# KaffinPX/neptune-core

Hardware: AMD Instinct MI355X
Metric: STARK proofs verified/sec (whole node) + Tip5 perms/sec vs VALU roofline (higher is better)
Workload: dtype u64 (Goldilocks mod p; XFE = cubic extension)

## Files before the change

neptune-core_amd/csrc/stark_kernels.hip:

```cpp
#include <hip/hip_ext.h>

#include <atomic>
#include <cstdlib>

#include "../../include/nhip_challenge_id.h"
#include "kernels.hpp"
#include "proof_codec.hpp"
#include "stark.hpp"
#include "stark_launch_plan.hpp"
#include "tip5_device.hpp"
#include "xfe.hpp"

namespace nhip {

#ifndef NHIP_LAT_PRIO
#define NHIP_LAT_PRIO 2
#endif
__device__ __forceinline__ void latency_priority() {
    if constexpr (NHIP_LAT_PRIO > 0) __builtin_amdgcn_s_setprio(NHIP_LAT_PRIO);
}
__device__ uint32_t g_batches_done;
struct AgePrio {
    uint32_t seq, k;
};
__device__ __forceinline__ void age_priority(AgePrio a, int base) {
    bool old = false;
    if (a.k) {
        const uint32_t done = __builtin_amdgcn_readfirstlane(
            __hip_atomic_load(&g_batches_done, __ATOMIC_RELAXED, __HIP_MEMORY_SCOPE_AGENT));
        old = (int32_t)(a.seq - done) < (int32_t)a.k;
    }
    switch (base + (old ? 1 : 0)) {
        case 0: break;
        case 1: __builtin_amdgcn_s_setprio(1); break;
        case 2: __builtin_amdgcn_s_setprio(2); break;
        default: __builtin_amdgcn_s_setprio(3); break;
// ... 213 lines not shown
                if (f + e < nwords) xs[xcur + f + e] = s[0];
                if (f + 4 + e < nwords) xs[xcur + f + 4 + e] = s[1];
                if (r2 && f + 8 + e < nwords) xs[xcur + f + 8 + e] = s[2];
                tip5_permute_quad(s, cq, rck, e, lds.lut);
            }
            xcur += nwords;
        } else {
            const uint64_t bound = op.arg;
            uint32_t got = 0;
            while (got < op.n) {
                const uint64_t v0 = from_mont(s[0]), v1 = from_mont(s[1]), v2 = from_mont(s[2]);
                tip5_permute_quad(s, cq, rck, e, lds.lut);
                const bool ok0 = v0 != GL_P - 1, ok1 = v1 != GL_P - 1, ok2 = r2 && v2 != GL_P - 1;
                const uint64_t b0 = __ballot(ok0), b1 = __ballot(ok1), b2 = __ballot(ok2);
                const uint32_t bits = ((uint32_t)(b0 >> qb) & 0xFu) | (((uint32_t)(b1 >> qb) & 0xFu) << 4) |
                                      (((uint32_t)(b2 >> qb) & 0x3u) << 8);
                auto put = [&](bool ok, uint32_t w, uint64_t v) {
                    const uint32_t rank = __popc(bits & ((1u << w) - 1u));
                    if (ok && got + rank < op.n) idx_out[icur + got + rank] = (uint32_t)((v & 0xFFFFFFFFull) % bound);
                };
                put(ok0, e, v0);
                put(ok1, 4 + e, v1);
                put(ok2, 8 + e, v2);
                got += __popc(bits);
            }
            icur += op.n;
        }
    }
}

#ifndef NHIP_ROWS_WAVES
#define NHIP_ROWS_WAVES 5
#endif
template <bool MW>
__global__ void __launch_bounds__(256, NHIP_ROWS_WAVES) k_hash_rows(const uint64_t* __restrict__ words, const ProofDesc* __restrict__ desc,
                                                   uint32_t n_proofs, uint32_t k, StarkDims dims,
                                                   uint64_t* __restrict__ dig, const uint32_t* __restrict__ fail,
                                                   AgePrio age) {
    age_priority(age, 0);
    __shared__ Tip5Lds lds;
    tip5_lds_init(lds);
    const uint32_t tree = blockIdx.y;
    const uint32_t width = tree == 0 ? dims.num_main : (tree == 1 ? 3 * dims.num_aux : 3 * dims.num_quot_seg);
    for (uint64_t t = blockIdx.x * (uint64_t)blockDim.x + threadIdx.x; t < (uint64_t)n_proofs * k;
         t += (uint64_t)gridDim.x * blockDim.x) {
        const uint32_t p = (uint32_t)(t / k), j = (uint32_t)(t % k);
        if (fail[p]) continue;
        const ProofDesc& d = desc[p];
        const uint64_t base = (tree == 0 ? d.main_rows_off : (tree == 1 ? d.aux_rows_off : d.quot_rows_off)) +
                              (uint64_t)j * width;
        const uint64_t* __restrict__ row = words + base;
        uint64_t s[16];
#pragma unroll
        for (int q = 0; q < 16; ++q) s[q] = 0;
        const uint32_t nchunks = width / TIP5_RATE + 1;
        for (uint32_t c = 0; c < nchunks; ++c) {
            const uint32_t pos = c * TIP5_RATE;
            const bool last = c + 1 == nchunks;
            if (!last) {
#pragma unroll
                for (int q = 0; q < TIP5_RATE; ++q) s[q] = word_mont<MW>(row[pos + q]);
            } else {
                const uint32_t rem = width - pos;
#pragma unroll
                for (int q = 0; q < TIP5_RATE; ++q) {
                    const uint32_t qq = (uint32_t)q;
                    s[q] = qq < rem ? word_mont<MW>(row[pos + qq]) : (qq == rem ? MONT_ONE : 0ull);
                }
            }
            tip5_rounds_0_3(s, lds.lut);
            tip5_last_sbox(s, lds.lut);
            if (!last) tip5_last_mds<10, 16>(s);
            else tip5_last_mds<0, 5>(s);
        }
        uint64_t* __restrict__ o = dig + (((uint64_t)p * 3 + tree) * k + j) * 5;
#pragma unroll
        for (int q = 0; q < 5; ++q) o[q] = s[q];
    }
}

template <bool MW>
__device__ __forceinline__ void hash_rows_wide_body(uint32_t bx, uint32_t tree, const Tip5Lds& t5,
                                                    const uint64_t* __restrict__ words,
                                                    const ProofDesc* __restrict__ desc, uint32_t n_proofs,
                                                    uint32_t k, StarkDims dims, uint64_t* __restrict__ dig,
                                                    const uint32_t* __restrict__ fail) {
    const uint32_t width = tree == 0 ? dims.num_main : (tree == 1 ? 3 * dims.num_aux : 3 * dims.num_quot_seg);
    const uint32_t e = threadIdx.x & 15u;
    const uint64_t t = ((uint64_t)bx * blockDim.x + threadIdx.x) >> 4;
    if (t >= (uint64_t)n_proofs * k) return;
    const uint32_t p = (uint32_t)(t / k), j = (uint32_t)(t % k);
    if (fail[p]) return;
    const ProofDesc& d = desc[p];
    const uint64_t* __restrict__ row =
        words + (tree == 0 ? d.main_rows_off : (tree == 1 ? d.aux_rows_off : d.quot_rows_off)) + (uint64_t)j * width;
    uint64_t rcs[TIP5_ROUNDS];
#pragma unroll
    for (int r = 0; r < TIP5_ROUNDS; ++r) rcs[r] = c_tip5_rc_raw[r * 16 + e];
    const uint32_t nchunks = width / TIP5_RATE + 1;
    auto chunk_word = [&](uint32_t c) -> uint64_t {
        const uint32_t pos = c * TIP5_RATE;
        if (c + 1 < nchunks) return e < TIP5_RATE ? word_mont<MW>(row[pos + e]) : 0ull;
        const uint32_t rem = width - pos;
// ... 299 lines not shown
                                               unsigned long long* __restrict__ perm_counter) {
    latency_priority();
    mp_plan_body<B>(blockIdx.x, blockIdx.y, words, desc, n_proofs, k, trees_per_proof, dig, idx_all, plan, fail,
                    perm_counter);
}

struct LcwTree {
    uint64_t* nodes;
    uint32_t max_len;
};

template <bool MW>
__device__ __forceinline__ void lcw_node(const uint64_t* __restrict__ words, const ProofDesc& d,
                                         const uint64_t* __restrict__ mine, uint32_t v, uint32_t L, uint64_t o[5]) {
    if (v >= L) {
        const uint64_t off = d.last_cw_off + 3ull * (v - L);
        o[0] = word_mont<MW>(words[off]);
        o[1] = word_mont<MW>(words[off + 1]);
        o[2] = word_mont<MW>(words[off + 2]);
        o[3] = 0;
        o[4] = 0;
    } else {
#pragma unroll
        for (int q = 0; q < 5; ++q) o[q] = mine[5ull * v + q];
    }
}

#ifndef NHIP_MP_WAVES
#define NHIP_MP_WAVES 6
#endif
#ifndef NHIP_MP_WAVES_SMALL
#define NHIP_MP_WAVES_SMALL 7
#endif
template <int WAVES, bool MW>
__global__ void __launch_bounds__(256, WAVES) k_mp_hash(const uint64_t* __restrict__ words, const uint64_t* __restrict__ dig,
                                                 MpPlan plan, uint32_t lvl, uint32_t mp_blocks,
                                                 const ProofDesc* __restrict__ desc, uint32_t n_proofs,
                                                 const uint32_t* __restrict__ fail, LcwTree lcw, AgePrio age) {
    __shared__ Tip5Lds t5;
    __shared__ uint64_t s_base[MP_SHARDS + 1];
    __shared__ uint32_t s_cnt[MP_SHARDS];
    age_priority(age, NHIP_MP_PRIO);
    const bool is_lcw = blockIdx.x >= mp_blocks;
    if (!is_lcw) {
        if (threadIdx.x < MP_SHARDS) {
            s_base[threadIdx.x] = plan.shard_base[lvl * MP_SHARDS + threadIdx.x];
            s_cnt[threadIdx.x] = plan.counter[lvl * MP_SHARDS + threadIdx.x];
        }
        if (threadIdx.x == 0)
            s_base[MP_SHARDS] = plan.shard_base[(lvl + 1) * MP_SHARDS - 1] + plan.shard_cap[(lvl + 1) * MP_SHARDS - 1];
    }
    tip5_lds_init(t5);
    uint64_t s[16];
    uint64_t* o = nullptr;
    bool work = false;
    if (is_lcw) {
        const uint32_t per = lcw.max_len >> (lvl + 1);
        const uint64_t q = (uint64_t)(blockIdx.x - mp_blocks) * blockDim.x + threadIdx.x;
        const uint32_t p = (uint32_t)(q / per), i = (uint32_t)(q % per);
        if (p < n_proofs && !(fail[p] & FAIL_DECODE)) {
            const ProofDesc& d = desc[p];
            const uint32_t L = d.last_cw_n;
            if (i < (L >> (lvl + 1))) {
                const uint32_t v = (L >> (lvl + 1)) + i;
                uint64_t* mine = lcw.nodes + (uint64_t)p * lcw.max_len * 5;
                lcw_node<MW>(words, d, mine, 2 * v, L, s);
                lcw_node<MW>(words, d, mine, 2 * v + 1, L, s + 5);
                o = mine + 5ull * v;
                work = true;
            }
        }
    } else {
        const uint64_t g = s_base[0] + (uint64_t)blockIdx.x * blockDim.x + threadIdx.x;
        if (g < s_base[MP_SHARDS]) {
            uint32_t sh = 0;
#pragma unroll
            for (uint32_t q = 1; q < MP_SHARDS; ++q) sh += g >= s_base[q] ? 1u : 0u;
            if (g - s_base[sh] < s_cnt[sh]) {
                const uint64_t lc = plan.ops[2 * g], rc = plan.ops[2 * g + 1];
                if (lc != MPS_NONE) {
                    mp_load<MW>(lc, words, dig, plan.arena, s);
                    mp_load<MW>(rc, words, dig, plan.arena, s + 5);
                    o = plan.arena + 5 * g;
                    work = true;
                }
            }
        }
    }
    if (!work) return;
    tip5_hash_pair_digest(s, t5.lut);
#pragma unroll
    for (int q = 0; q < 5; ++q) o[q] = s[q];
}

template <bool MW>
__device__ __forceinline__ uint64_t mp_load_word(uint64_t code, uint32_t e, const uint64_t* __restrict__ words,
                                                 const uint64_t* __restrict__ dig, const uint64_t* __restrict__ arena) {
    const uint64_t t = code >> 62, v = code & MPS_MASK;
    if (t == MPS_ARENA) return arena[5 * v + e];
    if (t == MPS_DIG) return dig[5 * v + e];
    if (t == MPS_AUTH) return word_mont<MW>(words[v + e]);
    return e < 3 ? word_mont<MW>(words[v + e]) : 0ull;
}

template <bool MW>
__device__ __forceinline__ uint64_t lcw_node_word(const uint64_t* __restrict__ words, const ProofDesc& d,
                                                  const uint64_t* __restrict__ mine, uint32_t v, uint32_t L, uint32_t e) {
    if (v >= L) return e < 3 ? word_mont<MW>(words[d.last_cw_off + 3ull * (v - L) + e]) : 0ull;
    return mine[5ull * v + e];
}

template <bool MW>
__global__ void __launch_bounds__(256) k_mp_hash_wide(const uint64_t* __restrict__ words,
                                                      const uint64_t* __restrict__ dig, MpPlan plan, uint32_t lvl,
                                                      uint64_t mp_rows, const ProofDesc* __restrict__ desc,
                                                      uint32_t n_proofs, const uint32_t* __restrict__ fail, LcwTree lcw) {
    latency_priority();
    __shared__ Tip5Lds t5;
    __shared__ uint64_t s_base[MP_SHARDS + 1];
    __shared__ uint32_t s_cnt[MP_SHARDS];
    if (threadIdx.x < MP_SHARDS) {
        s_base[threadIdx.x] = plan.shard_base[lvl * MP_SHARDS + threadIdx.x];
        s_cnt[threadIdx.x] = plan.counter[lvl * MP_SHARDS + threadIdx.x];
// ... 827 lines not shown
        hipLaunchKernelGGL(k_fs_rows_small<MW>, dim3(p.fs_grid), dim3(p.fs_block), 0, sa, b.words, b.desc, b.ops, n, b.xs,
                           b.idx, b.fail, age_sponge, p.fs_blocks, p.rows_gx, k, b.dims, b.dig);
    else if (p.fs_form == FS_PAIR)
        hipLaunchKernelGGL((k_fs_replay_wide<true, MW>), dim3(p.fs_grid), dim3(p.fs_block), 0, sa, b.words, b.desc, b.ops,
                           n, b.xs, b.idx, b.fail, age_sponge);
    else if (p.fs_form == FS_QUAD)
        hipLaunchKernelGGL(k_fs_replay_quad<MW>, dim3(p.fs_grid), dim3(p.fs_block), 0, sa, b.words, b.desc, b.ops, n,
                           b.xs, b.idx, b.fail, age_sponge);
    else
        hipLaunchKernelGGL((k_fs_replay_wide<false, MW>), dim3(p.fs_grid), dim3(p.fs_block), 0, sa, b.words, b.desc,
                           b.ops, n, b.xs, b.idx, b.fail, age_sponge);
    pad(sa);
    mark(EV_FS_DONE, sa);
    if (p.fused_plan_fri) {
        mark(EV_FRI_START, sa);
        hipLaunchKernelGGL(k_plan_fri_small<MW>, dim3(n * p.plan_groups + n), dim3(256), 0, sa, b.words, b.desc, n, k,
                           tpp, p.plan_groups, b.dig, b.idx, b.mp, b.fail, b.counters + CNT_MP_SKIPPED, b.dims, b.xs,
                           b.xdom);
    } else if (p.plan_block == 128) {
        hipLaunchKernelGGL(k_mp_plan<128>, dim3(n, p.plan_groups), dim3(128), 0, sa, b.words, b.desc, n, k, tpp, b.dig,
                           b.idx, b.mp, b.fail, b.counters + CNT_MP_SKIPPED);
    } else {
        hipLaunchKernelGGL(k_mp_plan<256>, dim3(n, p.plan_groups), dim3(256), 0, sa, b.words, b.desc, n, k, tpp, b.dig,
                           b.idx, b.mp, b.fail, b.counters + CNT_MP_SKIPPED);
    }
    pad(sa);
    mark(EV_PLAN_DONE, sa);
    if (!p.fused_fs_rows) {
        hipEvent_t r0 = p.rows_timed ? tm->rev[0] : nullptr, r1 = p.rows_timed ? tm->rev[1] : nullptr;
        if (p.rows_wide)
            launch_ev(k_hash_rows_wide<MW>, dim3(p.rows_grid, 3), dim3(256), 0, st, r0, r1, b.words, b.desc, n, k, b.dims,
                      b.dig, b.fail);
        else
            launch_ev(k_hash_rows<MW>, dim3(p.rows_grid, 3), dim3(256), 0, st, r0, r1, b.words, b.desc, n, k, b.dims,
                      b.dig, b.fail, age);
    }
    pad(st);
    mark(EV_ROWS_DONE, st);
    auto fri = [&](hipStream_t s) {
        hipLaunchKernelGGL(k_fri<MW>, dim3(n), dim3(256), 0, s, b.words, b.desc, n, b.dims, b.xs, b.idx, b.xdom, b.fail);
    };
    if (p.fri_on_main) {
        if (!p.fused_plan_fri) {
            wait(st, EV_FS_DONE);
            mark(EV_FRI_START, st);
            fri(st);
            pad(st);
        }
        mark(EV_FRI_DONE, st);
    }
    wait(st, EV_PLAN_DONE);
    auto aux_chain = [&]() {
        mark(EV_AUX_RELEASE, st);
        if (!p.fri_on_main) wait(sa, EV_AUX_RELEASE);
        mark(EV_AUX_START, sa);
        if (p.ood_block == 1024) {
            if (p.ood_global_slots) ood(k_ood_air<1024, MW, true>);
            else ood(k_ood_air<1024, MW, false>);
        } else {
            if (p.ood_global_slots) ood(k_ood_air<256, MW, true>);
            else ood(k_ood_air<256, MW, false>);
        }
        pad(sa);
        mark(EV_OOD_DONE, sa);
        if (p.fri_on_main) {
            wait(sa, EV_FRI_DONE);
        } else {
            fri(sa);
            mark(EV_FRI_DONE, sa);
        }
        hipLaunchKernelGGL(k_deep_rows8<MW>, dim3(n), dim3(256), deep_rows8_lds_bytes(b.dims), sa, b.words, b.desc, n,
                           b.dims, b.xs, b.xdom, b.ood, b.fail);
        pad(sa);
        mark(EV_DEEP_DONE, sa);
    };
    auto climb = [&](const HashStep& h) {
        launch_ev(k_mp_climb<MW>, dim3(h.grid, tpp + 1), dim3(MP_CLIMB_THREADS), 0, st, timed(h, 0), timed(h, 1), b.words,
                  b.dig, b.mp, tpp, b.desc, n, (const uint32_t*)b.fail, lcw, h.level);
    };
    for (uint32_t s = 0; s < p.n_steps; ++s) {
        if (s == p.aux_release_step) aux_chain();
        const HashStep& h = p.steps[s];
        switch (h.kind) {
            case HashKind::Climb: climb(h); break;
            case HashKind::Tail: {
                TailCaps caps{};
                for (uint32_t t = 0; t < MP_TAIL_LEVELS_MAX; ++t) caps.cap[t] = p.tail_caps[t];
                launch_ev(k_mp_hash_tail<MW>, dim3(h.grid), dim3(MP_TAIL_THREADS), 0, st, timed(h, 0), timed(h, 1), b.words,
                          b.dig, b.mp, h.level, p.hash_levels, caps, b.desc, n, (const uint32_t*)b.fail, lcw);
                break;
            }
            case HashKind::Wide:
                launch_ev(k_mp_hash_wide<MW>, dim3(h.grid), dim3(256), 0, st, timed(h, 0), timed(h, 1), b.words, b.dig,
                          b.mp, h.level, h.arg, b.desc, n, (const uint32_t*)b.fail, lcw);
                break;
            case HashKind::Level7:
                launch_ev((k_mp_hash<NHIP_MP_WAVES_SMALL, MW>), dim3(h.grid), dim3(256), 0, st, timed(h, 0), timed(h, 1),
                          b.words, b.dig, b.mp, h.level, (uint32_t)h.arg, b.desc, n, (const uint32_t*)b.fail, lcw, age);
                break;
            case HashKind::Level6:
                launch_ev((k_mp_hash<NHIP_MP_WAVES, MW>), dim3(h.grid), dim3(256), 0, st, timed(h, 0), timed(h, 1),
                          b.words, b.dig, b.mp, h.level, (uint32_t)h.arg, b.desc, n, (const uint32_t*)b.fail, lcw, age);
                break;
        }
    }
    if (p.one_climb) pad(st);
    if (p.aux_release_step == p.n_steps) aux_chain();
    mark(EV_HASH_DONE, st);
    if (p.roots_one_launch) {
        hipLaunchKernelGGL(k_roots_verdicts_small<MW>, dim3(p.roots_grid), dim3(ROOTS_ONE_WG), 0, st, b.words, b.desc,
                           b.dig, b.mp, p.n_records, tpp, k, b.fail, n, lcw, b.verdicts);
        mark(EV_ROOTS_DONE, st);
    } else {
        hipLaunchKernelGGL(k_mp_roots<MW>, dim3(p.roots_grid), dim3(256), 0, st, b.words, b.desc, b.dig, b.mp,
                           p.n_records, tpp, k, b.fail, n, lcw);
        pad(st);
        mark(EV_ROOTS_DONE, st);
        wait(st, EV_DEEP_DONE);
        hipLaunchKernelGGL(k_verdicts, dim3(p.verdicts_grid), dim3(256), 0, st, b.fail, n, b.verdicts);
    }
    mark(EV_VERDICTS, st);
    return hipGetLastError();
}

hipError_t launch_stark_phases(const StarkBatchDev& b, hipStream_t st, hipStream_t sa, StarkPhaseTimer* tm) {
    return b.D.mont_words ? launch_phases<true>(b, st, sa, tm) : launch_phases<false>(b, st, sa, tm);
}

template <bool MW>
static hipError_t set_attributes() {
    for (const void* f : {(const void*)k_ood_air<256, MW, false>, (const void*)k_ood_air<256, MW, true>,
                          (const void*)k_ood_air<1024, MW, false>, (const void*)k_ood_air<1024, MW, true>}) {
        const hipError_t e = hipFuncSetAttribute(f, hipFuncAttributeMaxDynamicSharedMemorySize, AIR_LDS_BUDGET);
        if (e != hipSuccess) return e;
// ... 12 lines not shown
```

neptune-core_amd/csrc/stark_launch_plan.hpp:

```cpp
#pragma once
#include <cstdint>
#include <cstdlib>

#include "ab_env.hpp"
#include "kernels.hpp"

namespace nhip {

static constexpr uint32_t MP_CLIMB_MAX_PROOFS = 32;
static constexpr uint32_t ROWS_WIDE_MAX_PROOFS = 32;
static constexpr uint32_t OOD_WIDE_MAX_PROOFS = 64;
static constexpr uint32_t FS_PAIR_MAX_PROOFS = 512;
static constexpr uint32_t FS_QUAD_MIN_PROOFS = 2048;
static constexpr uint32_t FS_QUAD_WG = 256;
static constexpr uint32_t MP_SMALL_MAX_PROOFS = 4096;
static constexpr uint64_t MP_WIDE_MAX_OPS = 48 * 1024;
#ifndef NHIP_MP_TAIL_MAX_OPS
#define NHIP_MP_TAIL_MAX_OPS 256
#endif
static constexpr uint64_t MP_TAIL_MAX_OPS = NHIP_MP_TAIL_MAX_OPS;
static constexpr uint32_t CLIMB_FROM_MIN_LEVELS = 24;
static constexpr uint64_t CLIMB_FROM_OPS_DEFAULT = 4096;
static constexpr uint32_t CLIMB_FROM_MIN_REST = 3;
static constexpr uint32_t AUX_AFTER_LEVEL_DEFAULT = 0;
static constexpr uint32_t AGE_PRIO_OLDEST = 2;
static constexpr uint32_t AGE_PRIO_MIN_PROOFS = 2048;

enum FsForm { FS_ROW = 0, FS_PAIR = 1, FS_QUAD = 2 };

struct LaunchKnobs {
    uint32_t ood_wide_max = OOD_WIDE_MAX_PROOFS;
    uint32_t rows_wide_max = ROWS_WIDE_MAX_PROOFS;
    uint32_t quad_wg = FS_QUAD_WG;
    uint32_t quad_min = FS_QUAD_MIN_PROOFS;
    int fs_form_init = -1;
    int64_t age_prio = -1;
    bool age_prio_fs = false;
    bool fuse_fs_rows = true;
    bool fuse_plan_fri = true;
    uint32_t mp_small_max = MP_SMALL_MAX_PROOFS;
    uint32_t climb_max = MP_CLIMB_MAX_PROOFS;
    uint32_t aux_after_level = AUX_AFTER_LEVEL_DEFAULT;
    int pad_packets = 0;
};

inline unsigned long ab_unsigned(const char* name, unsigned long dflt) {
    const char* e = ab_env(name);
    return e ? std::strtoul(e, nullptr, 10) : dflt;
}

inline LaunchKnobs launch_knobs_from_env() {
    LaunchKnobs kn;
    kn.ood_wide_max = (uint32_t)ab_unsigned("NHIP_OOD_WIDE_MAX", kn.ood_wide_max);
    kn.rows_wide_max = (uint32_t)ab_unsigned("NHIP_ROWS_WIDE_MAX", kn.rows_wide_max);
    const uint32_t w = (uint32_t)ab_unsigned("NHIP_QUAD_WG", FS_QUAD_WG);
    kn.quad_wg = (w >= 64 && w <= 1024 && w % 64 == 0) ? w : FS_QUAD_WG;
    kn.quad_min = (uint32_t)ab_unsigned("NHIP_FS_QUAD_MIN", kn.quad_min);
    if (const char* v = ab_env("NHIP_FS_FORM"))
        kn.fs_form_init = v[0] == 'q' ? (int)FS_QUAD : v[0] == 'p' ? (int)FS_PAIR : v[0] == 'r' ? (int)FS_ROW : -1;
    kn.age_prio = (int64_t)ab_unsigned("NHIP_AGE_PRIO", (unsigned long)-1);
    if (const char* e = ab_env("NHIP_AGE_PRIO_FS")) kn.age_prio_fs = e[0] == '1';
    if (const char* e = ab_env("NHIP_FUSE_SMALL")) kn.fuse_fs_rows = e[0] != '0';
    if (const char* e = ab_env("NHIP_FUSE_PLAN_FRI")) kn.fuse_plan_fri = e[0] != '0';
    kn.mp_small_max = (uint32_t)ab_unsigned("NHIP_MP_SMALL_MAX", kn.mp_small_max);
    kn.climb_max = (uint32_t)ab_unsigned("NHIP_CLIMB_MAX", kn.climb_max);
    kn.aux_after_level = (uint32_t)ab_unsigned("NHIP_AUX_AFTER_LEVEL", kn.aux_after_level);
    kn.pad_packets = (int)ab_unsigned("NHIP_PAD_PACKETS", 0);
    return kn;
}
inline const LaunchKnobs& launch_knobs() {
    static const LaunchKnobs kn = launch_knobs_from_env();
    return kn;
}

static constexpr uint32_t event_bit(StarkEvent e) { return 1u << (int)e; }
static constexpr uint32_t CROSS_STREAM_EVENTS = event_bit(EV_FORK) | event_bit(EV_DECODED) | event_bit(EV_FS_DONE) |
                                                event_bit(EV_PLAN_DONE) | event_bit(EV_FRI_DONE) |
                                                event_bit(EV_AUX_RELEASE) | event_bit(EV_DEEP_DONE);
static constexpr uint32_t ALL_EVENTS = (1u << STARK_EVENTS) - 1;

struct LaunchInput {
    uint32_t n, k, max_R;
    uint32_t mp_levels;
    const uint64_t* mp_cap_host;
    uint32_t max_lcw;
    bool global_slots;
    uint32_t air_block;
    bool two_streams;
    bool phase_marks;
    bool launch_events;
    bool hash_events;
    int fs_form_forced;
    int64_t climb_from_forced;
};

enum class HashKind : uint8_t {
    Level6,
    Level7,
    Wide,
    Tail,
// ... 155 lines not shown
```

neptune-core_amd/csrc/tip5_device.hpp:

```cpp
#pragma once
#include "goldilocks.hpp"
#include "tip5_constants.h"

namespace nhip {

static constexpr int TIP5_STATE = 16;
static constexpr int TIP5_RATE = 10;
static constexpr int TIP5_ROUNDS = 5;
static constexpr uint64_t MONT_ONE = 0x00000000FFFFFFFFull;

__constant__ static uint64_t c_tip5_rc_raw[80] = {
#define NHIP_RC(i) TIP5_RC_RAW[i]
    NHIP_RC(0), NHIP_RC(1), NHIP_RC(2), NHIP_RC(3), NHIP_RC(4), NHIP_RC(5), NHIP_RC(6), NHIP_RC(7),
    NHIP_RC(8), NHIP_RC(9), NHIP_RC(10), NHIP_RC(11), NHIP_RC(12), NHIP_RC(13), NHIP_RC(14), NHIP_RC(15),
    NHIP_RC(16), NHIP_RC(17), NHIP_RC(18), NHIP_RC(19), NHIP_RC(20), NHIP_RC(21), NHIP_RC(22), NHIP_RC(23),
    NHIP_RC(24), NHIP_RC(25), NHIP_RC(26), NHIP_RC(27), NHIP_RC(28), NHIP_RC(29), NHIP_RC(30), NHIP_RC(31),
    NHIP_RC(32), NHIP_RC(33), NHIP_RC(34), NHIP_RC(35), NHIP_RC(36), NHIP_RC(37), NHIP_RC(38), NHIP_RC(39),
    NHIP_RC(40), NHIP_RC(41), NHIP_RC(42), NHIP_RC(43), NHIP_RC(44), NHIP_RC(45), NHIP_RC(46), NHIP_RC(47),
    NHIP_RC(48), NHIP_RC(49), NHIP_RC(50), NHIP_RC(51), NHIP_RC(52), NHIP_RC(53), NHIP_RC(54), NHIP_RC(55),
    NHIP_RC(56), NHIP_RC(57), NHIP_RC(58), NHIP_RC(59), NHIP_RC(60), NHIP_RC(61), NHIP_RC(62), NHIP_RC(63),
    NHIP_RC(64), NHIP_RC(65), NHIP_RC(66), NHIP_RC(67), NHIP_RC(68), NHIP_RC(69), NHIP_RC(70), NHIP_RC(71),
    NHIP_RC(72), NHIP_RC(73), NHIP_RC(74), NHIP_RC(75), NHIP_RC(76), NHIP_RC(77), NHIP_RC(78), NHIP_RC(79),
#undef NHIP_RC
};

__constant__ static uint64_t c_tip5_rck_raw[80] = {
#define NHIP_RC(i) (TIP5_RC_RAW[i] + 0xFFFFFFFFull)
    NHIP_RC(0), NHIP_RC(1), NHIP_RC(2), NHIP_RC(3), NHIP_RC(4), NHIP_RC(5), NHIP_RC(6), NHIP_RC(7),
    NHIP_RC(8), NHIP_RC(9), NHIP_RC(10), NHIP_RC(11), NHIP_RC(12), NHIP_RC(13), NHIP_RC(14), NHIP_RC(15),
    NHIP_RC(16), NHIP_RC(17), NHIP_RC(18), NHIP_RC(19), NHIP_RC(20), NHIP_RC(21), NHIP_RC(22), NHIP_RC(23),
    NHIP_RC(24), NHIP_RC(25), NHIP_RC(26), NHIP_RC(27), NHIP_RC(28), NHIP_RC(29), NHIP_RC(30), NHIP_RC(31),
    NHIP_RC(32), NHIP_RC(33), NHIP_RC(34), NHIP_RC(35), NHIP_RC(36), NHIP_RC(37), NHIP_RC(38), NHIP_RC(39),
    NHIP_RC(40), NHIP_RC(41), NHIP_RC(42), NHIP_RC(43), NHIP_RC(44), NHIP_RC(45), NHIP_RC(46), NHIP_RC(47),
    NHIP_RC(48), NHIP_RC(49), NHIP_RC(50), NHIP_RC(51), NHIP_RC(52), NHIP_RC(53), NHIP_RC(54), NHIP_RC(55),
    NHIP_RC(56), NHIP_RC(57), NHIP_RC(58), NHIP_RC(59), NHIP_RC(60), NHIP_RC(61), NHIP_RC(62), NHIP_RC(63),
// ... 180 lines not shown
#endif
template <int NIN, int OBEG, int OEND, int G>
__device__ __forceinline__ void mds_fold_groups(const uint32_t* lo, const uint32_t* hi,
                                                const uint64_t* __restrict__ rck, uint64_t* out) {
    constexpr int N = (OEND - OBEG) < G ? (OEND - OBEG) : G;
    mds_fold_outputs<NIN, OBEG, N>(lo, hi, rck, out);
    if constexpr (OBEG + N < OEND) {
        __builtin_amdgcn_sched_barrier(0);
        mds_fold_groups<NIN, OBEG + N, OEND, G>(lo, hi, rck, out + N);
    }
}

template <int NIN, int OBEG = 0, int OEND = 16, int G = 16>
__device__ __forceinline__ void mds_ark_fold(uint64_t s[16], const uint64_t* __restrict__ rck) {
    uint32_t lo[NIN], hi[NIN];
#pragma unroll
    for (int j = 0; j < NIN; ++j) {
        lo[j] = (uint32_t)s[j];
        hi[j] = (uint32_t)(s[j] >> 32);
    }
    uint64_t out[OEND - OBEG];
    mds_fold_groups<NIN, OBEG, OEND, G>(lo, hi, rck, out);
#pragma unroll
    for (int o = 0; o < OEND - OBEG; ++o) s[OBEG + o] = out[o];
}

template <int G = NHIP_SPONGE_MDS_GROUP>
__device__ __forceinline__ void mds_ark(uint64_t s[16], const uint64_t* __restrict__ rc,
                                        const uint64_t* __restrict__ rck) {
    (void)rc;
    mds_ark_fold<16, 0, 16, G>(s, rck);
}

__device__ __forceinline__ void tip5_permute_raw(uint64_t s[16], const uint8_t* __restrict__ lut) {
#pragma unroll 1
    for (int r = 0; r < TIP5_ROUNDS; ++r) {
#pragma unroll
        for (int i = 0; i < 4; ++i) s[i] = split_and_lookup(lut, s[i]);
        pow7_12(s + 4);
        mds_ark(s, c_tip5_rc_raw + r * 16, c_tip5_rck_raw + r * 16);
    }
}


__host__ __device__ constexpr uint64_t tip5_rck0_fixed(int i) {
    uint64_t k = TIP5_RC_RAW[i] + 0xFFFFFFFFull;
    for (int j = 10; j < 16; ++j) k += (uint64_t)TIP5_MDS[(i - j) & 15] * 0xFFFFFFFFull;
    return k;
}
constexpr bool tip5_rck0_fixed_in_range() {
    for (int i = 0; i < 16; ++i)
        if (tip5_rck0_fixed(i) >= 0xFFF0000000000000ull || tip5_rck0_fixed(i) < TIP5_RC_RAW[i]) return false;
    return true;
}
static_assert(tip5_rck0_fixed_in_range(), "round-0 FixedLength accumulator start below 2^64 - 2^52");
__constant__ static uint64_t c_tip5_rck0_fixed[16] = {
    tip5_rck0_fixed(0),  tip5_rck0_fixed(1),  tip5_rck0_fixed(2),  tip5_rck0_fixed(3),
    tip5_rck0_fixed(4),  tip5_rck0_fixed(5),  tip5_rck0_fixed(6),  tip5_rck0_fixed(7),
    tip5_rck0_fixed(8),  tip5_rck0_fixed(9),  tip5_rck0_fixed(10), tip5_rck0_fixed(11),
    tip5_rck0_fixed(12), tip5_rck0_fixed(13), tip5_rck0_fixed(14), tip5_rck0_fixed(15),
};

__device__ __forceinline__ void tip5_hash_pair_digest(uint64_t s[16], const uint8_t* __restrict__ lut) {
#pragma unroll
    for (int i = 0; i < 4; ++i) s[i] = split_and_lookup(lut, s[i]);
#pragma unroll
    for (int g = 4; g < 10; g += 3) {
        uint64_t x2[3], x4[3], x3[3];
        pow7_mul<3>(s + g, s + g, x2);
        pow7_mul<3>(x2, x2, x4);
        pow7_mul<3>(s + g, x2, x3);
        pow7_mul<3>(x3, x4, s + g);
    }
    mds_ark_fold<10, 0, 16, NHIP_PAIR_MDS_GROUP>(s, c_tip5_rck0_fixed);
#pragma unroll 1
    for (int r = 1; r < TIP5_ROUNDS - 1; ++r) {
#pragma unroll
        for (int i = 0; i < 4; ++i) s[i] = split_and_lookup(lut, s[i]);
        pow7_12(s + 4);
        mds_ark<NHIP_PAIR_MDS_GROUP>(s, c_tip5_rc_raw + r * 16, c_tip5_rck_raw + r * 16);
    }
#pragma unroll
    for (int i = 0; i < 4; ++i) s[i] = split_and_lookup(lut, s[i]);
    pow7_12(s + 4);
    mds_ark_fold<16, 0, 5, NHIP_PAIR_MDS_GROUP>(s, c_tip5_rck_raw + (TIP5_ROUNDS - 1) * 16);
}

__device__ __forceinline__ void tip5_rounds_0_3(uint64_t s[16], const uint8_t* __restrict__ lut) {
#pragma unroll 1
    for (int r = 0; r < TIP5_ROUNDS - 1; ++r) {
#pragma unroll
        for (int i = 0; i < 4; ++i) s[i] = split_and_lookup(lut, s[i]);
        pow7_12(s + 4);
        mds_ark(s, c_tip5_rc_raw + r * 16, c_tip5_rck_raw + r * 16);
    }
}
__device__ __forceinline__ void tip5_last_sbox(uint64_t s[16], const uint8_t* __restrict__ lut) {
#pragma unroll
    for (int i = 0; i < 4; ++i) s[i] = split_and_lookup(lut, s[i]);
    pow7_12(s + 4);
}
template <int OBEG, int OEND>
__device__ __forceinline__ void tip5_last_mds(uint64_t s[16]) {
    mds_ark_fold<16, OBEG, OEND, NHIP_SPONGE_MDS_GROUP>(s, c_tip5_rck_raw + (TIP5_ROUNDS - 1) * 16);
}
template <int OBEG, int OEND>
__device__ __forceinline__ void tip5_last_round(uint64_t s[16], const uint8_t* __restrict__ lut) {
    tip5_last_sbox(s, lut);
    tip5_last_mds<OBEG, OEND>(s);
}

}

namespace nhip {

__device__ __forceinline__ uint64_t mds_reduce_ark_lat(uint64_t al, uint64_t ah, uint64_t nq) {
    const uint64_t w = (uint64_t)(uint32_t)(al >> 32) + (uint32_t)ah;
    const uint32_t sh = (uint32_t)(ah >> 32) + (uint32_t)(w >> 32);
    const uint64_t slo = ((uint64_t)(uint32_t)w << 32) | (uint32_t)al;
    const uint64_t res = slo + (uint64_t)sh * 0xFFFFFFFFull;
    const uint64_t y = res + (res < slo ? GL_EPS : 0ull);
    const uint64_t x1 = y + nq;
    return x1 + (x1 > y ? GL_P : 0ull);
}

__device__ __forceinline__ uint64_t mds_reduce_fold(uint64_t al, uint64_t ah) {
    unsigned int k;
// ... 195 lines not shown
```

Baseline: 472,900.

## Compute Tip5 MDS layer with int8 MFMA byte-plane decomposition in hash kernels

Splits each 64-bit Tip5 state word into signed byte planes and evaluates the circulant MDS matrix via i8 32x32x32 MFMA instructions against signed-digit tiles of the MDS coefficients, then recombines plane results with shifted multiply-adds before the existing fold reduction. The goal is to move MDS multiply work off the VALU onto the matrix cores. It is enabled for row hashing when the proof count reaches a threshold, and for Merkle-path hashing only in an A/B build with an env flag. The planes variants lower launch-bound waves to make room for the extra vector registers holding the tiles, which may reduce occupancy.

```diff
diff --git a/neptune-core_amd/csrc/stark_kernels.hip b/neptune-core_amd/csrc/stark_kernels.hip
--- a/neptune-core_amd/csrc/stark_kernels.hip
+++ b/neptune-core_amd/csrc/stark_kernels.hip
@@ -2,6 +2,7 @@
 
 #include <atomic>
 #include <cstdlib>
+#include <type_traits>
 
 #include "../../include/nhip_challenge_id.h"
 #include "kernels.hpp"
@@ -281,14 +282,19 @@
 #ifndef NHIP_ROWS_WAVES
 #define NHIP_ROWS_WAVES 5
 #endif
-template <bool MW>
-__global__ void __launch_bounds__(256, NHIP_ROWS_WAVES) k_hash_rows(const uint64_t* __restrict__ words, const ProofDesc* __restrict__ desc,
+#ifndef NHIP_ROWS_WAVES_PLANES
+#define NHIP_ROWS_WAVES_PLANES 4
+#endif
+template <bool MW, bool PLANES>
+__global__ void __launch_bounds__(256, PLANES ? NHIP_ROWS_WAVES_PLANES : NHIP_ROWS_WAVES) k_hash_rows(const uint64_t* __restrict__ words, const ProofDesc* __restrict__ desc,
                                                    uint32_t n_proofs, uint32_t k, StarkDims dims,
                                                    uint64_t* __restrict__ dig, const uint32_t* __restrict__ fail,
                                                    AgePrio age) {
     age_priority(age, 0);
     __shared__ Tip5Lds lds;
     tip5_lds_init(lds);
+    std::conditional_t<PLANES, Tip5Planes, Tip5NoPlanes> pl;
+    if constexpr (PLANES) tip5_planes_init(pl);
     const uint32_t tree = blockIdx.y;
     const uint32_t width = tree == 0 ? dims.num_main : (tree == 1 ? 3 * dims.num_aux : 3 * dims.num_quot_seg);
     for (uint64_t t = blockIdx.x * (uint64_t)blockDim.x + threadIdx.x; t < (uint64_t)n_proofs * k;
@@ -317,7 +323,7 @@
                     s[q] = qq < rem ? word_mont<MW>(row[pos + qq]) : (qq == rem ? MONT_ONE : 0ull);
                 }
             }
-            tip5_rounds_0_3(s, lds.lut);
+            tip5_rounds_0_3(s, lds.lut, pl);
             tip5_last_sbox(s, lds.lut);
             if (!last) tip5_last_mds<10, 16>(s);
             else tip5_last_mds<0, 5>(s);
@@ -683,8 +689,11 @@
 #ifndef NHIP_MP_WAVES_SMALL
 #define NHIP_MP_WAVES_SMALL 7
 #endif
-template <int WAVES, bool MW>
-__global__ void __launch_bounds__(256, WAVES) k_mp_hash(const uint64_t* __restrict__ words, const uint64_t* __restrict__ dig,
+#ifndef NHIP_MP_WAVES_PLANES
+#define NHIP_MP_WAVES_PLANES 4
+#endif
+template <int WAVES, bool MW, bool PLANES>
+__global__ void __launch_bounds__(256, PLANES ? NHIP_MP_WAVES_PLANES : WAVES) k_mp_hash(const uint64_t* __restrict__ words, const uint64_t* __restrict__ dig,
                                                  MpPlan plan, uint32_t lvl, uint32_t mp_blocks,
                                                  const ProofDesc* __restrict__ desc, uint32_t n_proofs,
                                                  const uint32_t* __restrict__ fail, LcwTree lcw, AgePrio age) {
@@ -702,6 +711,8 @@
             s_base[MP_SHARDS] = plan.shard_base[(lvl + 1) * MP_SHARDS - 1] + plan.shard_cap[(lvl + 1) * MP_SHARDS - 1];
     }
     tip5_lds_init(t5);
+    std::conditional_t<PLANES, Tip5Planes, Tip5NoPlanes> pl;
+    if constexpr (PLANES) tip5_planes_init(pl);
     uint64_t s[16];
     uint64_t* o = nullptr;
     bool work = false;
@@ -739,7 +750,7 @@
         }
     }
     if (!work) return;
-    tip5_hash_pair_digest(s, t5.lut);
+    tip5_hash_pair_digest(s, t5.lut, pl);
 #pragma unroll
     for (int q = 0; q < 5; ++q) o[q] = s[q];
 }
@@ -1633,8 +1644,8 @@
             launch_ev(k_hash_rows_wide<MW>, dim3(p.rows_grid, 3), dim3(256), 0, st, r0, r1, b.words, b.desc, n, k, b.dims,
                       b.dig, b.fail);
         else
-            launch_ev(k_hash_rows<MW>, dim3(p.rows_grid, 3), dim3(256), 0, st, r0, r1, b.words, b.desc, n, k, b.dims,
-                      b.dig, b.fail, age);
+            launch_ev(n >= kn.rows_planes_min ? k_hash_rows<MW, true> : k_hash_rows<MW, false>, dim3(p.rows_grid, 3), dim3(256), 0,
+                      st, r0, r1, b.words, b.desc, n, k, b.dims, b.dig, b.fail, age);
     }
     pad(st);
     mark(EV_ROWS_DONE, st);
@@ -1675,6 +1686,12 @@
         pad(sa);
         mark(EV_DEEP_DONE, sa);
     };
+#ifdef NHIP_AB_BUILD
+    constexpr bool MP_PLANES_BUILT = true;
+#else
+    constexpr bool MP_PLANES_BUILT = false;
+#endif
+    const bool mp_planes = MP_PLANES_BUILT && kn.mds_planes_mp;
     auto climb = [&](const HashStep& h) {
         launch_ev(k_mp_climb<MW>, dim3(h.grid, tpp + 1), dim3(MP_CLIMB_THREADS), 0, st, timed(h, 0), timed(h, 1), b.words,
                   b.dig, b.mp, tpp, b.desc, n, (const uint32_t*)b.fail, lcw, h.level);
@@ -1696,11 +1713,11 @@
                           b.mp, h.level, h.arg, b.desc, n, (const uint32_t*)b.fail, lcw);
                 break;
             case HashKind::Level7:
-                launch_ev((k_mp_hash<NHIP_MP_WAVES_SMALL, MW>), dim3(h.grid), dim3(256), 0, st, timed(h, 0), timed(h, 1),
+                launch_ev(mp_planes ? k_mp_hash<NHIP_MP_WAVES_SMALL, MW, MP_PLANES_BUILT> : k_mp_hash<NHIP_MP_WAVES_SMALL, MW, false>, dim3(h.grid), dim3(256), 0, st, timed(h, 0), timed(h, 1),
                           b.words, b.dig, b.mp, h.level, (uint32_t)h.arg, b.desc, n, (const uint32_t*)b.fail, lcw, age);
                 break;
             case HashKind::Level6:
-                launch_ev((k_mp_hash<NHIP_MP_WAVES, MW>), dim3(h.grid), dim3(256), 0, st, timed(h, 0), timed(h, 1),
+                launch_ev(mp_planes ? k_mp_hash<NHIP_MP_WAVES, MW, MP_PLANES_BUILT> : k_mp_hash<NHIP_MP_WAVES, MW, false>, dim3(h.grid), dim3(256), 0, st, timed(h, 0), timed(h, 1),
                           b.words, b.dig, b.mp, h.level, (uint32_t)h.arg, b.desc, n, (const uint32_t*)b.fail, lcw, age);
                 break;
         }
diff --git a/neptune-core_amd/csrc/stark_launch_plan.hpp b/neptune-core_amd/csrc/stark_launch_plan.hpp
--- a/neptune-core_amd/csrc/stark_launch_plan.hpp
+++ b/neptune-core_amd/csrc/stark_launch_plan.hpp
@@ -13,6 +13,7 @@
 static constexpr uint32_t FS_PAIR_MAX_PROOFS = 512;
 static constexpr uint32_t FS_QUAD_MIN_PROOFS = 2048;
 static constexpr uint32_t FS_QUAD_WG = 256;
+static constexpr uint32_t ROWS_PLANES_MIN_PROOFS = 512;
 static constexpr uint32_t MP_SMALL_MAX_PROOFS = 4096;
 static constexpr uint64_t MP_WIDE_MAX_OPS = 48 * 1024;
 #ifndef NHIP_MP_TAIL_MAX_OPS
@@ -42,6 +43,8 @@
     uint32_t climb_max = MP_CLIMB_MAX_PROOFS;
     uint32_t aux_after_level = AUX_AFTER_LEVEL_DEFAULT;
     int pad_packets = 0;
+    uint32_t rows_planes_min = ROWS_PLANES_MIN_PROOFS;
+    bool mds_planes_mp = false;
 };
 
 inline unsigned long ab_unsigned(const char* name, unsigned long dflt) {
@@ -66,6 +69,8 @@
     kn.climb_max = (uint32_t)ab_unsigned("NHIP_CLIMB_MAX", kn.climb_max);
     kn.aux_after_level = (uint32_t)ab_unsigned("NHIP_AUX_AFTER_LEVEL", kn.aux_after_level);
     kn.pad_packets = (int)ab_unsigned("NHIP_PAD_PACKETS", 0);
+    kn.rows_planes_min = (uint32_t)ab_unsigned("NHIP_ROWS_PLANES_MIN", kn.rows_planes_min);
+    if (const char* e = ab_env("NHIP_MDS_PLANES_MP")) kn.mds_planes_mp = e[0] == '1';
     return kn;
 }
 inline const LaunchKnobs& launch_knobs() {
diff --git a/neptune-core_amd/csrc/tip5_device.hpp b/neptune-core_amd/csrc/tip5_device.hpp
--- a/neptune-core_amd/csrc/tip5_device.hpp
+++ b/neptune-core_amd/csrc/tip5_device.hpp
@@ -1,6 +1,7 @@
 #pragma once
 #include "goldilocks.hpp"
 #include "tip5_constants.h"
+#include "tip5_mds_planes.hpp"
 
 namespace nhip {
 
@@ -247,13 +248,148 @@
     mds_ark_fold<16, 0, 16, G>(s, rck);
 }
 
-__device__ __forceinline__ void tip5_permute_raw(uint64_t s[16], const uint8_t* __restrict__ lut) {
+typedef int tip5_v4i __attribute__((ext_vector_type(4)));
+typedef int tip5_v16i __attribute__((ext_vector_type(16)));
+
+struct Tip5PlanesTable {
+    uint32_t w[3 * 64 * 4];
+};
+constexpr Tip5PlanesTable tip5_planes_table() {
+    Tip5PlanesTable tb{};
+    for (int e = 0; e < 3; ++e)
+        for (int l = 0; l < 64; ++l)
+            for (int t = 0; t < 16; ++t)
+                tb.w[(e * 64 + l) * 4 + t / 4] |= (uint32_t)(uint8_t)(int8_t)planes_tile_byte(e, l, t) << (8 * (t % 4));
+    return tb;
+}
+__constant__ static Tip5PlanesTable c_tip5_planes_tiles = tip5_planes_table();
+
+__constant__ static uint64_t c_tip5_rckp_raw[80] = {
+#define NHIP_RC(i) planes_start(TIP5_RC_RAW[i] + 0xFFFFFFFFull)
+    NHIP_RC(0), NHIP_RC(1), NHIP_RC(2), NHIP_RC(3), NHIP_RC(4), NHIP_RC(5), NHIP_RC(6), NHIP_RC(7),
+    NHIP_RC(8), NHIP_RC(9), NHIP_RC(10), NHIP_RC(11), NHIP_RC(12), NHIP_RC(13), NHIP_RC(14), NHIP_RC(15),
+    NHIP_RC(16), NHIP_RC(17), NHIP_RC(18), NHIP_RC(19), NHIP_RC(20), NHIP_RC(21), NHIP_RC(22), NHIP_RC(23),
+    NHIP_RC(24), NHIP_RC(25), NHIP_RC(26), NHIP_RC(27), NHIP_RC(28), NHIP_RC(29), NHIP_RC(30), NHIP_RC(31),
+    NHIP_RC(32), NHIP_RC(33), NHIP_RC(34), NHIP_RC(35), NHIP_RC(36), NHIP_RC(37), NHIP_RC(38), NHIP_RC(39),
+    NHIP_RC(40), NHIP_RC(41), NHIP_RC(42), NHIP_RC(43), NHIP_RC(44), NHIP_RC(45), NHIP_RC(46), NHIP_RC(47),
+    NHIP_RC(48), NHIP_RC(49), NHIP_RC(50), NHIP_RC(51), NHIP_RC(52), NHIP_RC(53), NHIP_RC(54), NHIP_RC(55),
+    NHIP_RC(56), NHIP_RC(57), NHIP_RC(58), NHIP_RC(59), NHIP_RC(60), NHIP_RC(61), NHIP_RC(62), NHIP_RC(63),
+    NHIP_RC(64), NHIP_RC(65), NHIP_RC(66), NHIP_RC(67), NHIP_RC(68), NHIP_RC(69), NHIP_RC(70), NHIP_RC(71),
+    NHIP_RC(72), NHIP_RC(73), NHIP_RC(74), NHIP_RC(75), NHIP_RC(76), NHIP_RC(77), NHIP_RC(78), NHIP_RC(79),
+#undef NHIP_RC
+};
+
+struct Tip5Planes {
+    tip5_v4i tile[3];
+    int32_t k0, k8, k16, k24;
+};
+__device__ __forceinline__ void tip5_planes_init(Tip5Planes& pl) {
+    const uint32_t lane = __builtin_amdgcn_mbcnt_hi(~0u, __builtin_amdgcn_mbcnt_lo(~0u, 0u));
+    const tip5_v4i* tb = (const tip5_v4i*)c_tip5_planes_tiles.w;
+#pragma unroll
+    for (int e = 0; e < 3; ++e) {
+        pl.tile[e] = tb[e * 64 + lane];
+        asm volatile("" : "+v"(pl.tile[e]));
+    }
+    asm("v_mov_b32 %0, 1" : "=v"(pl.k0));
+    asm("s_mov_b32 %0, 0x100" : "=s"(pl.k8));
+    asm("s_mov_b32 %0, 0x10000" : "=s"(pl.k16));
+    asm("s_mov_b32 %0, 0x1000000" : "=s"(pl.k24));
+}
+
+template <int Q>
+__device__ __forceinline__ tip5_v16i planes_cq(const Tip5Planes& pl, const tip5_v4i* plane) {
+    tip5_v16i c = {0, 0, 0, 0, 0, 0, 0, 0, 0, 0, 0, 0, 0, 0, 0, 0};
+#pragma unroll
+    for (int e = 0; e < 3; ++e)
+        if (Q - e >= 0 && Q - e <= 7) c = __builtin_amdgcn_mfma_i32_32x32x32_i8(pl.tile[e], plane[Q - e], c, 0, 0, 0);
+    return c;
+}
+
+__device__ __forceinline__ int64_t planes_mad(int32_t c, int32_t k, int64_t a) { return (int64_t)c * (int64_t)k + a; }
+
+__host__ __device__ constexpr int planes_order(int k) {
+    constexpr int o[10] = {0, 1, 2, 3, 9, 8, 4, 5, 6, 7};
+    return o[k];
+}
+template <int K>
+__device__ __forceinline__ void planes_step(const Tip5Planes& pl, const tip5_v4i* plane, const tip5_v16i& c,
+                                            const uint64_t* __restrict__ rckp, int64_t* al, int64_t* t, uint32_t* hb) {
+    constexpr int Q = planes_order(K);
+    tip5_v16i next;
+    if constexpr (K < 9) next = planes_cq<planes_order(K + 1)>(pl, plane);
+#pragma unroll
+    for (int i = 0; i < 16; ++i) {
+        if constexpr (Q == 0) al[i] = planes_mad(c[i], pl.k0, (int64_t)rckp[i]);
+        if constexpr (Q == 1) al[i] = planes_mad(c[i], pl.k8, al[i]);
+        if constexpr (Q == 2) al[i] = planes_mad(c[i], pl.k16, al[i]);
+        if constexpr (Q == 3) al[i] = planes_mad(c[i], pl.k24, al[i]);
+        if constexpr (Q == 9) hb[i] = ((uint32_t)c[i] << 8) + (uint32_t)PLANES_HB_BIAS;
+        if constexpr (Q == 8) t[i] = (int64_t)(((uint64_t)(hb[i] + (uint32_t)c[i]) << 32) | (uint32_t)((uint64_t)al[i] >> 32));
+        if constexpr (Q == 4) t[i] = planes_mad(c[i], pl.k0, t[i]);
+        if constexpr (Q == 5) t[i] = planes_mad(c[i], pl.k8, t[i]);
+        if constexpr (Q == 6) t[i] = planes_mad(c[i], pl.k16, t[i]);
+        if constexpr (Q == 7) t[i] = planes_mad(c[i], pl.k24, t[i]);
+    }
+    if constexpr (K < 9) {
+        __builtin_amdgcn_sched_barrier(0);
+        planes_step<K + 1>(pl, plane, next, rckp, al, t, hb);
+    }
+}
+
+__device__ __forceinline__ void mds_ark_planes(uint64_t s[16], const uint64_t* __restrict__ rckp, const Tip5Planes& pl) {
+    tip5_v4i plane[8];
+#pragma unroll
+    for (int m = 0; m < 4; ++m)
+#pragma unroll
+        for (int h = 0; h < 2; ++h) {
+            uint32_t w[4];
+#pragma unroll
+            for (int b = 0; b < 4; ++b) w[b] = (uint32_t)(s[4 * m + b] >> (32 * h)) ^ 0x80808080u;
+            const uint32_t a0 = __builtin_amdgcn_perm(w[1], w[0], 0x05010400u);
+            const uint32_t a1 = __builtin_amdgcn_perm(w[1], w[0], 0x07030602u);
+            const uint32_t c0 = __builtin_amdgcn_perm(w[3], w[2], 0x05010400u);
+            const uint32_t c1 = __builtin_amdgcn_perm(w[3], w[2], 0x07030602u);
+            plane[4 * h + 0][m] = (int)__builtin_amdgcn_perm(c0, a0, 0x05040100u);
+            plane[4 * h + 1][m] = (int)__builtin_amdgcn_perm(c0, a0, 0x07060302u);
+            plane[4 * h + 2][m] = (int)__builtin_amdgcn_perm(c1, a1, 0x05040100u);
+            plane[4 * h + 3][m] = (int)__builtin_amdgcn_perm(c1, a1, 0x07060302u);
+        }
+    int64_t al[16], t[16];
+    uint32_t hb[16];
+    planes_step<0>(pl, plane, planes_cq<0>(pl, plane), rckp, al, t, hb);
+    uint32_t sh[16], e[16];
+    uint64_t slo[16], w[16];
+#pragma unroll
+    for (int i = 0; i < 16; ++i) {
+        sh[i] = (uint32_t)((uint64_t)t[i] >> 32);
+        slo[i] = ((uint64_t)t[i] << 32) | (uint32_t)al[i];
+    }
+#pragma unroll
+    for (int i = 0; i < 16; i += 4) mds_fold4(sh + i, slo + i, w + i, e + i);
+#pragma unroll
+    for (int i = 0; i < 16; ++i) s[i] = w[i] - e[i];
+}
+
+struct Tip5NoPlanes {};
+template <class PL>
+inline constexpr bool tip5_is_planes = false;
+template <>
+inline constexpr bool tip5_is_planes<Tip5Planes> = true;
+template <int G, class PL>
+__device__ __forceinline__ void mds_ark_round(uint64_t s[16], int r, const PL& pl) {
+    if constexpr (tip5_is_planes<PL>) mds_ark_planes(s, c_tip5_rckp_raw + r * 16, pl);
+    else mds_ark<G>(s, c_tip5_rc_raw + r * 16, c_tip5_rck_raw + r * 16);
+}
+
+template <class PL = Tip5NoPlanes>
+__device__ __forceinline__ void tip5_permute_raw(uint64_t s[16], const uint8_t* __restrict__ lut, const PL& pl = PL{}) {
 #pragma unroll 1
     for (int r = 0; r < TIP5_ROUNDS; ++r) {
 #pragma unroll
         for (int i = 0; i < 4; ++i) s[i] = split_and_lookup(lut, s[i]);
         pow7_12(s + 4);
-        mds_ark(s, c_tip5_rc_raw + r * 16, c_tip5_rck_raw + r * 16);
+        mds_ark_round<NHIP_SPONGE_MDS_GROUP>(s, r, pl);
     }
 }
 
@@ -276,7 +412,8 @@
     tip5_rck0_fixed(12), tip5_rck0_fixed(13), tip5_rck0_fixed(14), tip5_rck0_fixed(15),
 };
 
-__device__ __forceinline__ void tip5_hash_pair_digest(uint64_t s[16], const uint8_t* __restrict__ lut) {
+template <class PL = Tip5NoPlanes>
+__device__ __forceinline__ void tip5_hash_pair_digest(uint64_t s[16], const uint8_t* __restrict__ lut, const PL& pl = PL{}) {
 #pragma unroll
     for (int i = 0; i < 4; ++i) s[i] = split_and_lookup(lut, s[i]);
 #pragma unroll
@@ -293,7 +430,7 @@
 #pragma unroll
         for (int i = 0; i < 4; ++i) s[i] = split_and_lookup(lut, s[i]);
         pow7_12(s + 4);
-        mds_ark<NHIP_PAIR_MDS_GROUP>(s, c_tip5_rc_raw + r * 16, c_tip5_rck_raw + r * 16);
+        mds_ark_round<NHIP_PAIR_MDS_GROUP>(s, r, pl);
     }
 #pragma unroll
     for (int i = 0; i < 4; ++i) s[i] = split_and_lookup(lut, s[i]);
@@ -301,13 +438,14 @@
     mds_ark_fold<16, 0, 5, NHIP_PAIR_MDS_GROUP>(s, c_tip5_rck_raw + (TIP5_ROUNDS - 1) * 16);
 }
 
-__device__ __forceinline__ void tip5_rounds_0_3(uint64_t s[16], const uint8_t* __restrict__ lut) {
+template <class PL = Tip5NoPlanes>
+__device__ __forceinline__ void tip5_rounds_0_3(uint64_t s[16], const uint8_t* __restrict__ lut, const PL& pl = PL{}) {
 #pragma unroll 1
     for (int r = 0; r < TIP5_ROUNDS - 1; ++r) {
 #pragma unroll
         for (int i = 0; i < 4; ++i) s[i] = split_and_lookup(lut, s[i]);
         pow7_12(s + 4);
-        mds_ark(s, c_tip5_rc_raw + r * 16, c_tip5_rck_raw + r * 16);
+        mds_ark_round<NHIP_SPONGE_MDS_GROUP>(s, r, pl);
     }
 }
 __device__ __forceinline__ void tip5_last_sbox(uint64_t s[16], const uint8_t* __restrict__ lut) {
diff --git a/neptune-core_amd/csrc/tip5_mds_planes.hpp b/neptune-core_amd/csrc/tip5_mds_planes.hpp
--- /dev/null
+++ b/neptune-core_amd/csrc/tip5_mds_planes.hpp
@@ -0,0 +1,80 @@
+#pragma once
+#include <stdint.h>
+
+#include "tip5_constants.h"
+
+#if defined(__HIPCC__) || defined(__CUDACC__)
+#define NHIP_PLANES_HD __host__ __device__
+#else
+#define NHIP_PLANES_HD
+#endif
+
+namespace nhip {
+
+static constexpr uint64_t PLANES_P = 0xFFFFFFFF00000001ull;
+static constexpr int32_t PLANES_HB_BIAS = 1 << 29;
+static constexpr uint64_t PLANES_START_MIN = 1ull << 45;
+static constexpr uint64_t PLANES_START_MAX = 0ull - (1ull << 45);
+
+NHIP_PLANES_HD constexpr int mds_digit(int k, int e) {
+    const int m = (int)TIP5_MDS[k];
+    const int b0 = m & 0xFF;
+    const int e0 = b0 < 128 ? b0 : b0 - 256;
+    const int m1 = (m - e0) >> 8;
+    const int b1 = m1 & 0xFF;
+    const int e1 = b1 < 128 ? b1 : b1 - 256;
+    const int e2 = (m1 - e1) >> 8;
+    return e == 0 ? e0 : e == 1 ? e1 : e2;
+}
+constexpr bool mds_digits_in_range() {
+    for (int k = 0; k < 16; ++k) {
+        const int e0 = mds_digit(k, 0), e1 = mds_digit(k, 1), e2 = mds_digit(k, 2);
+        if (e0 < -128 || e0 > 127 || e1 < -128 || e1 > 127 || e2 < 0 || e2 > 1) return false;
+        if (e0 + 256 * e1 + 65536 * e2 != (int)TIP5_MDS[k]) return false;
+    }
+    return true;
+}
+static_assert(mds_digits_in_range(), "every MDS coefficient is e0 + 2^8 e1 + 2^16 e2 in signed bytes");
+
+constexpr int64_t planes_cq_bound() {
+    int64_t b = 0;
+    for (int k = 0; k < 16; ++k) {
+        int64_t a = 0;
+        for (int e = 0; e < 3; ++e) a += mds_digit(k, e) < 0 ? -mds_digit(k, e) : mds_digit(k, e);
+        b += 128 * a;
+    }
+    return b;
+}
+static_assert(planes_cq_bound() < (1 << 20), "|C_q| < 2^20");
+
+constexpr uint64_t planes_mod_p(unsigned __int128 x) { return (uint64_t)(x % PLANES_P); }
+constexpr uint64_t planes_mds_sum() {
+    uint64_t s = 0;
+    for (int k = 0; k < 16; ++k) s += TIP5_MDS[k];
+    return s;
+}
+static constexpr uint64_t PLANES_OFFSET =
+    planes_mod_p((unsigned __int128)0x8080808080808080ull * planes_mds_sum());
+static constexpr uint64_t PLANES_BIAS = planes_mod_p((unsigned __int128)1 << 93);
+
+NHIP_PLANES_HD constexpr uint64_t planes_start(uint64_t k) {
+    return (uint64_t)(((unsigned __int128)(k % PLANES_P) + PLANES_OFFSET + (PLANES_P - PLANES_BIAS)) % PLANES_P);
+}
+constexpr bool planes_start_in_range(uint64_t k) {
+    return planes_start(k) >= PLANES_START_MIN && planes_start(k) < PLANES_START_MAX;
+}
+constexpr bool planes_starts_in_range() {
+    for (int i = 0; i < 80; ++i)
+        if (!planes_start_in_range(TIP5_RC_RAW[i] + 0xFFFFFFFFull)) return false;
+    return true;
+}
+static_assert(planes_starts_in_range(), "al = start + L neither under- nor overflows for any Tip5 round constant");
+
+NHIP_PLANES_HD constexpr int planes_tile_byte(int e, int l, int t) {
+    const int row = l & 31, half = l >> 5;
+    if (((row >> 2) & 1) != half) return 0;
+    const int i = (row & 3) + 4 * (row >> 3);
+    return mds_digit((i - t) & 15, e);
+}
+
+}
```

Result: faster. 498,000, median of 6 (+5.3%).
